# vliu15/3d-brain-tumor-segmentation

Hardware: AMD Instinct MI355X
Metric: training volumes/sec (2ch x 128^3) (higher is better)
Workload: dtype f32; 1 GPU; BASELINE configs[1]: 2ch x 128^3, batch 1 per GPU, fp32, full fwd+bwd with Dice+KL+L2 VAE loss + Dice metric + TF-form Adam; CLI-default model (base_filters=32, depth=4, groups=8, reduction=8; 42,174,773 params); parallelism=dp1, global_batch=1

## Files before the change

3d-brain-tumor-segmentation_amd/csrc/conv_igemm.hip:

```cpp
#include <stdlib.h>
#include "common.h"
#include "conv_plan.h"

#define MAXSLOT 8

int bts_prof_on();
void bts_prof_begin(int sym, double flops, hipStream_t stream);
void bts_prof_end(hipStream_t stream);

struct IgemmParams {
  const float* x;
  const float* wp;
  const float* bias;
  float* y;
  int N, Di, Hi, Wi, Cin, ldx;
  int Do, Ho, Wo;
  int Cout, ldy, Npad, KG;
  int ODa, OHa, OWa;
  int os, ooz, ooy, oox;
  int s, loz, loy, lox;
  int IZ, IY, IX;
  int lgTX, lgTY, TZ;
  int ntz, nty, ntx;
  int ntaps, flags;
// ... 1622 lines not shown
  }
  r = conv_launch(c, ch, q, stream);
  if (r == BTS_OK && ch.second) r = conv_launch(c2, ch2, q2, stream);
  if (r == BTS_OK && gn_B) *gn_B = ch.gn_B;
  return r;
}

static int conv_call_of(int dir, int kind, int N, int D, int H, int W, int Cin, int ldx, int Cout, int ldy, int flags, ConvCall& c) {
  if (N <= 0 || D <= 0 || H <= 0 || W <= 0 || Cin <= 0 || Cout <= 0 || ldx < Cin || ldy < Cout) return BTS_ERR_SHAPE;
  if (kind == BTS_CONV_K3S2 && ((D | H | W) & 1)) return BTS_ERR_SHAPE;
  const bool same = kind == BTS_CONV_K1 || kind == BTS_CONV_K3S1, half = kind == BTS_CONV_K3S2;
  const int Df = same ? D : half ? D / 2 : 2 * D, Hf = same ? H : half ? H / 2 : 2 * H, Wf = same ? W : half ? W / 2 : 2 * W;
  c = ConvCall{};
  c.geo = kind == BTS_CONV_K1 ? GEO_K1 : kind == BTS_CONV_K3S1 ? GEO_S1 : half == (dir == 0) ? GEO_DOWN : GEO_UP;
  c.N = N;
  if (dir == 0) { c.Di = D; c.Hi = H; c.Wi = W; c.Do = Df; c.Ho = Hf; c.Wo = Wf; c.Cin = Cin; c.ldx = ldx; c.Cout = Cout; c.ldy = ldy; }
  else { c.Di = Df; c.Hi = Hf; c.Wi = Wf; c.Do = D; c.Ho = H; c.Wo = W; c.Cin = Cout; c.ldx = ldy; c.Cout = Cin; c.ldy = ldx; }
  if ((flags & BTS_CONV_FLAG_SIGMOID) && dir == 0) c.flags |= IG_FLAG_SIGMOID;
  if (flags & BTS_CONV_FLAG_ACCUM) c.flags |= IG_FLAG_ACCUM;
  return BTS_OK;
}
static void conv_query_view(ConvCall& c) { c.x16 = c.y16 = c.p2_16 = c.ws16 = 1; c.ws_bytes = LONG_MAX; }
static long conv_ws_query(int dir, int kind, int N, int D, int H, int W, int Cin, int Cout) {
  ConvCall c;
  ConvChoice ch;
  if (conv_call_of(dir, kind, N, D, H, W, Cin, Cin, Cout, Cout, 0, c) != BTS_OK) return -1;
  conv_query_view(c);
  if (c.geo == GEO_UP && upm_accept(c, ch) && ch.ws > 0) return ch.ws;
  if (igemm_accept(c, ch) != BTS_OK) return -1;
  long need = ch.ws;
  if (c.geo == GEO_S1) {
    const long wn = wino_ws_need(c), w3 = w3_ws_need(c);
    need = need > wn ? need : wn;
    need = need > w3 ? need : w3;
  }
  return need;
}

extern "C" int bts_conv3d_fwd(int kind, const float* x, const float* wp_fwd, const float* bias, float* y, void* workspace,
                              long workspace_bytes, int N, int D, int H, int W, int Cin, int ldx, int Cout, int ldy,
                              int flags, hipStream_t stream) {
  ConvCall c;
  const int r = conv_call_of(0, kind, N, D, H, W, Cin, ldx, Cout, ldy, flags, c);
  if (r != BTS_OK) return r;
  if (bias) c.flags |= IG_FLAG_BIAS;
  c.ws_bytes = workspace_bytes;
  ConvPtrs q = {};
  q.x = x; q.wp = wp_fwd; q.bias = bias; q.y = y; q.ws = workspace;
  return conv_run(c, q, stream);
}
extern "C" long bts_conv3d_fwd_workspace(int kind, int N, int D, int H, int W, int Cin, int Cout) {
  return conv_ws_query(0, kind, N, D, H, W, Cin, Cout);
}

extern "C" int bts_conv3d_bwd_data(int kind, const float* dy, const float* wp_bwd, float* dx, void* workspace,
                                   long workspace_bytes, int N, int D, int H, int W, int Cin, int lddx, int Cout, int lddy,
                                   int flags, hipStream_t stream) {
  ConvCall c;
  const int r = conv_call_of(1, kind, N, D, H, W, Cin, lddx, Cout, lddy, flags, c);
  if (r != BTS_OK) return r;
  c.ws_bytes = workspace_bytes;
  ConvPtrs q = {};
  q.x = dy; q.wp = wp_bwd; q.y = dx; q.ws = workspace;
  return conv_run(c, q, stream);
}
extern "C" long bts_conv3d_bwd_data_workspace(int kind, int N, int D, int H, int W, int Cin, int Cout) {
  return conv_ws_query(1, kind, N, D, H, W, Cin, Cout);
}

extern "C" int bts_conv3d_fwd_can_fuse(int N, int D, int H, int W, int Cin, int Cout) {
  ConvCall c;
  ConvChoice ch;
  if (conv_call_of(0, BTS_CONV_K3S1, N, D, H, W, Cin, Cin, Cout, Cout, 0, c) != BTS_OK) return 0;
  conv_query_view(c);
  c.second = CONV_Y2; c.ld2 = Cout;
  return igemm_accept(c, ch) == BTS_OK;
}
extern "C" int bts_conv3d_fwd_fused2(const float* x, const float* wp_fwd, const float* bias, float* y, const float* wp2,
                                     const float* bias2, float* y2, int N, int D, int H, int W, int Cin, int ldx, int Cout,
                                     int ldy, int ldy2, hipStream_t stream) {
  ConvCall c;
  if (conv_call_of(0, BTS_CONV_K3S1, N, D, H, W, Cin, ldx, Cout, ldy, 0, c) != BTS_OK || ldy2 < Cout || !wp2 || !y2) return BTS_ERR_SHAPE;
  if (bias) c.flags |= IG_FLAG_BIAS;
  c.second = CONV_Y2; c.ld2 = ldy2;
  ConvPtrs q = {};
  q.x = x; q.wp = wp_fwd; q.bias = bias; q.y = y; q.wp2 = wp2; q.bias2 = bias2; q.y2 = y2;
  return conv_run(c, q, stream);
}

extern "C" long bts_gn_workspace(int N, long V, int C, int G, int mode);
extern "C" int bts_gn_stats(const float* x, float* mean, float* rstd, void* workspace, long workspace_bytes, int N, long V, int C,
                            int G, int mode, float eps, hipStream_t stream);
static long gnfuse_partial_bytes(int N, int Do, int Ho, int Wo, int Cout) {
  const long tiles = (long)N * ((Do + 0) ) * ((Ho + 3) / 4) * ((Wo + 7) / 8);
  return tiles * ((npad32(Cout) + 31) / 32) * 2 * (long)sizeof(double) + 64;
}
extern "C" long bts_conv3d_fwd_gn_workspace(int kind, int N, int D, int H, int W, int Cin, int Cout, int G) {
  const long cw = bts_conv3d_fwd_workspace(kind, N, D, H, W, Cin, Cout);
  if (cw < 0) return -1;
  int Do = D, Ho = H, Wo = W;
  if (kind == BTS_CONV_K3S2) { Do = D / 2; Ho = H / 2; Wo = W / 2; }
  if (kind == BTS_CONV_K3S2T) { Do = 2 * D; Ho = 2 * H; Wo = 2 * W; }
  const long gw = bts_gn_workspace(N, (long)Do * Ho * Wo, Cout, G, BTS_GN_SLAB);
  if (gw < 0) return -1;
  const long fused = ((cw + 63) & ~63L) + gnfuse_partial_bytes(N, Do, Ho, Wo, Cout);
  return fused > gw ? fused : gw;
}
static int conv_fwd_gn_impl(int kind, const float* x, const float* wp, const float* bias, float* y, const float* wp2,
                            const float* bias2, float* y2, int ldy2, void* ws, long ws_bytes, int N, int D, int H, int W, int Cin,
                            int ldx, int Cout, int G, float eps, float* mean, float* rstd, hipStream_t stream) {
  if (G <= 0 || Cout % G != 0) return BTS_ERR_SHAPE;
  if (ws == nullptr || ws_bytes < bts_conv3d_fwd_gn_workspace(kind, N, D, H, W, Cin, Cout, G)) return BTS_ERR_WORKSPACE;
  ConvCall c;
  int r = conv_call_of(0, kind, N, D, H, W, Cin, ldx, Cout, Cout, 0, c);
  if (r != BTS_OK) return r;
  if (bias) c.flags |= IG_FLAG_BIAS;
  if (wp2 != nullptr) { c.second = CONV_Y2; c.ld2 = ldy2; }
  const long cw = (bts_conv3d_fwd_workspace(kind, N, D, H, W, Cin, Cout) + 63) & ~63L;
  c.G = G; c.ws_bytes = cw;
  ConvPtrs q = {};
  q.x = x; q.wp = wp; q.bias = bias; q.y = y; q.wp2 = wp2; q.bias2 = bias2; q.y2 = y2; q.ws = ws;
  q.gnp = reinterpret_cast<double*>(reinterpret_cast<char*>(ws) + cw);
  long gnB = 0;
  r = conv_run(c, q, stream, &gnB);
  if (r != BTS_OK) return r;
  const long V = (long)c.Do * c.Ho * c.Wo;
  if (gnB > 0) return bts_gn_finalize_partials_(q.gnp, mean, rstd, N * G, gnB, (double)V * Cout / G, eps, stream);
  return bts_gn_stats(y, mean, rstd, ws, ws_bytes, N, V, Cout, G, BTS_GN_SLAB, eps, stream);
}
extern "C" int bts_conv3d_fwd_gn(int kind, const float* x, const float* wp_fwd, const float* bias, float* y, void* workspace,
                                 long workspace_bytes, int N, int D, int H, int W, int Cin, int ldx, int Cout, int G, float eps,
                                 float* mean, float* rstd, hipStream_t stream) {
  if (N <= 0 || D <= 0 || H <= 0 || W <= 0 || Cin <= 0 || Cout <= 0 || ldx < Cin) return BTS_ERR_SHAPE;
  if (((uintptr_t)workspace) & 15) return BTS_ERR_ALIGN;
  return conv_fwd_gn_impl(kind, x, wp_fwd, bias, y, nullptr, nullptr, nullptr, 0, workspace, workspace_bytes, N, D, H, W, Cin, ldx,
                          Cout, G, eps, mean, rstd, stream);
}
extern "C" int bts_conv3d_fwd_fused2_gn(const float* x, const float* wp_fwd, const float* bias, float* y, const float* wp2,
                                        const float* bias2, float* y2, void* workspace, long workspace_bytes, int N, int D, int H,
                                        int W, int Cin, int ldx, int Cout, int ldy2, int G, float eps, float* mean, float* rstd,
                                        hipStream_t stream) {
  if (N <= 0 || D <= 0 || H <= 0 || W <= 0 || Cin <= 0 || Cout <= 0 || ldx < Cin || ldy2 < Cout || !wp2 || !y2) return BTS_ERR_SHAPE;
  if (((uintptr_t)workspace) & 15) return BTS_ERR_ALIGN;
  return conv_fwd_gn_impl(BTS_CONV_K3S1, x, wp_fwd, bias, y, wp2, bias2, y2, ldy2, workspace, workspace_bytes, N, D, H, W, Cin, ldx,
                          Cout, G, eps, mean, rstd, stream);
}

extern "C" long bts_conv3d_bwd_data_pair_workspace(int N, int D, int H, int W, int Cin, int Cout) {
  const long a = bts_conv3d_bwd_data_workspace(BTS_CONV_K3S1, N, D, H, W, Cin, Cout);
  const long b = bts_conv3d_bwd_data_workspace(BTS_CONV_K1, N, D, H, W, Cin, Cout);
  if (a < 0 || b < 0) return -1;
  return a > b ? a : b;
}
extern "C" int bts_conv3d_bwd_data_pair(const float* dy, const float* wp_bwd, const float* dy2, const float* wp2_bwd, float* dx,
                                        void* workspace, long workspace_bytes, int N, int D, int H, int W, int Cin, int lddx,
                                        int Cout, int lddy, int lddy2, int flags, hipStream_t stream) {
  ConvCall c;
  if (conv_call_of(1, BTS_CONV_K3S1, N, D, H, W, Cin, lddx, Cout, lddy, flags, c) != BTS_OK || lddy2 < Cout) return BTS_ERR_SHAPE;
  const long need = conv_ws_query(1, BTS_CONV_K3S1, N, D, H, W, Cin, Cout);
  if (need < 0) return BTS_ERR_SHAPE;
  c.ws_bytes = workspace_bytes;
  ConvPtrs q = {};
  q.x = dy; q.wp = wp_bwd; q.y = dx; q.ws = workspace;
  const bool fuse = need == 0 && (Cout % 8 == 0) && (lddy2 % 4 == 0) && ((((uintptr_t)dy2) & 15) == 0) && Cin > 4 &&
                    getenv("BTS_IGEMM_NOPAIR") == nullptr;
  if (fuse) {
    c.second = CONV_X2; c.ld2 = lddy2;
    q.x2 = dy2; q.wp2 = wp2_bwd;
    return conv_run(c, q, stream);
  }
  const int r = conv_run(c, q, stream);
  if (r != BTS_OK) return r;
  return bts_conv3d_bwd_data(BTS_CONV_K1, dy2, wp2_bwd, dx, workspace, workspace_bytes, N, D, H, W, Cin, lddx, Cout, lddy2,
                             flags | BTS_CONV_FLAG_ACCUM, stream);
}

static int conv_config_query(int dir, int kind, int N, int D, int H, int W, int Cin, int Cout) {
  ConvCall c;
  ConvChoice ch;
  int r = conv_call_of(dir, kind, N, D, H, W, Cin, Cin, Cout, Cout, 0, c);
  if (r != BTS_OK) return r;
  conv_query_view(c);
  r = igemm_accept(c, ch);
  return r != BTS_OK ? r : ch.sym;
}
extern "C" int bts_conv3d_fwd_config(int kind, int N, int D, int H, int W, int Cin, int Cout) {
  return conv_config_query(0, kind, N, D, H, W, Cin, Cout);
}
extern "C" int bts_conv3d_bwd_data_config(int kind, int N, int D, int H, int W, int Cin, int Cout) {
  return conv_config_query(1, kind, N, D, H, W, Cin, Cout);
}
extern "C" int bts_conv3d_kernel(int dir, int kind, int N, int D, int H, int W, int Cin, int ldx, int Cout, int ldy, int flags, int second,
                                 int ld2, int G, int aligned, long workspace_bytes) {
  ConvCall c;
  ConvChoice ch;
  int r = conv_call_of(dir != 0, kind, N, D, H, W, Cin, ldx, Cout, ldy, flags, c);
  if (r != BTS_OK) return r;
  if (second < 0 || second > CONV_X2 || G < 0) return BTS_ERR_SHAPE;
  if (second && (c.geo != GEO_S1 || ld2 < c.Cout * (second == CONV_Y2) + c.Cin * (second == CONV_X2))) return BTS_ERR_SHAPE;
  c.second = second; c.ld2 = second ? ld2 : 0; c.G = G;
  c.x16 = aligned & 1; c.y16 = (aligned >> 1) & 1; c.p2_16 = (aligned >> 2) & 1; c.ws16 = (aligned >> 3) & 1;
  c.ws_bytes = workspace_bytes < 0 ? LONG_MAX : workspace_bytes;
  r = conv_choose(c, ch);
  return r != BTS_OK ? r : ch.sym;
}
```

3d-brain-tumor-segmentation_amd/csrc/conv_wino3.hip:

```cpp
#include <stdio.h>
#include <stdlib.h>
#include <type_traits>
#include "common.h"
#include "conv_plan.h"
#include "wino_util.h"

int bts_prof_on();
void bts_prof_begin(int sym, double flops, hipStream_t stream);
void bts_prof_end(hipStream_t stream);

struct W3Params {
  const float* x;
  const float* up;
  const float* bias;
  float* y;
  int N, D, H, W, ldx, Cout, ldy, KG;
  int ntz, nty, ntx;
  int accum;
  double* gnp;
  int gn_G, gn_zt;
  int ksplit, kg_per, Npad;
  float* part;
  int nb, ntiles, tiles_per_xcd;
  int T;
};

#define W3S 12
#define W3SX 18
#define W3LX 20
#define W3NCOL (W3SX * 6 * 2)
#define W3PL (6 * W3LX * W3S)
#define W3BUF (8 * W3PL)
#define W3NSLOT 6
#define W3EX (4 * 4 * 4 * 64 * 4)
#define W3OFF(j, k) ((((j) * W3LX) + ((k) & 1) * 10 + ((k) >> 1)) * W3S)

__global__ __launch_bounds__(256, 1) void w3_kernel(const W3Params p) {
  extern __shared__ __attribute__((aligned(16))) float lds[];
  const int tid = threadIdx.x;
  const int lane = tid & 63;
  const int wave = __builtin_amdgcn_readfirstlane(tid >> 6);
  const int h = lane >> 5, l32 = lane & 31;
  const int ptx = l32 & 7, pty = (l32 >> 3) & 1, ptz = l32 >> 4;
  const int nb_ = p.nb;
  const int xcd_ = blockIdx.x & 7;
  const int seq0 = (blockIdx.x >> 3) * p.T;
  int tiles_left = p.ntiles - xcd_ * p.tiles_per_xcd;
  if (tiles_left > p.tiles_per_xcd) tiles_left = p.tiles_per_xcd;
  const int items_here = tiles_left * nb_;
  if (seq0 >= items_here) return;

  struct Item { int n, tz, ty, tx, cb; };
  auto decode = [&](int seq) {
    Item it;
    it.cb = seq % nb_;
    int b = xcd_ * p.tiles_per_xcd + seq / nb_;
    it.tx = b % p.ntx; b /= p.ntx;
    it.ty = b % p.nty; b /= p.nty;
    it.tz = b % p.ntz;
    it.n = b / p.ntz;
    return it;
  };
  auto advance = [&](Item& it) {
    if (++it.cb < nb_) return;
    it.cb = 0;
    if (++it.tx < p.ntx) return;
    it.tx = 0;
    if (++it.ty < p.nty) return;
    it.ty = 0;
    if (++it.tz < p.ntz) return;
    it.tz = 0;
    ++it.n;
  };

  const int s_q = tid & 1, s_vy = (tid >> 1) / W3SX, s_vx = (tid >> 1) - s_vy * W3SX;
  const bool s_on = tid < W3NCOL;
  const unsigned gcol = (unsigned)((s_vy * p.W + s_vx) * p.ldx + s_q * 4) * 4u;
  const unsigned gplane = (unsigned)(p.H * p.W * p.ldx) * 4u;
  const int lcol = (s_vy * W3LX + (s_vx & 1) * 10 + (s_vx >> 1)) * W3S + s_q * 4;
  __amdgpu_buffer_rsrc_t xr, wr, wr_n;
  unsigned goff[W3NSLOT];
  auto setup_x = [&](const Item& it) {
    const int iz0 = it.tz * 4 - 1, iy0 = it.ty * 4 - 1, ix0 = it.tx * 16 - 1;
    const float* xorg = p.x + ((((long)it.n * p.D + iz0) * p.H + iy0) * p.W + ix0) * (long)p.ldx;
    xr = __builtin_amdgcn_make_buffer_rsrc((void*)xorg, 0, 0x7fffffff, 0x00020000);
    const bool col_in = s_on && (unsigned)(iy0 + s_vy) < (unsigned)p.H && (unsigned)(ix0 + s_vx) < (unsigned)p.W;
#pragma unroll
    for (int i = 0; i < W3NSLOT; ++i) goff[i] = (col_in && (unsigned)(iz0 + i) < (unsigned)p.D) ? gcol + (unsigned)i * gplane : 0x80000000u;
  };
  auto wdesc = [&](const Item& it) {
    return __builtin_amdgcn_make_buffer_rsrc((void*)(p.up + (long)it.cb * p.KG * (64 * 256)), 0, 0x7fffffff, 0x00020000);
  };
  const __amdgpu_buffer_rsrc_t br =
      __builtin_amdgcn_make_buffer_rsrc((void*)p.bias, 0, (p.bias && p.ksplit <= 1) ? (unsigned)p.Cout * 4u : 0u, 0x00020000);
  auto bias_of = [&](const Item& it) {
    return __builtin_bit_cast(float, __builtin_amdgcn_raw_buffer_load_b32(br, tid < 32 ? (unsigned)(it.cb * 32 + tid) * 4u : 0x80000000u, 0, 0));
  };

  int st0 = 0, st1 = p.KG;
  if (p.ksplit > 1) {
    st0 = blockIdx.z * p.kg_per;
    st1 = st0 + p.kg_per;
    if (st1 > p.KG) st1 = p.KG;
  }

  const int offP = (ptz * 4 + wave) * W3PL + (2 * pty * W3LX + ptx) * W3S + h * 4;
  const unsigned wlane = (unsigned)((h * 32 + l32) * 16);
  const unsigned wwave = (unsigned)(wave * 16 * 1024);

  f32x16 acc[4][4];
  f32x4 pre[W3NSLOT];
  auto fetch = [&](unsigned soff) {
#pragma unroll
    for (int i = 0; i < W3NSLOT; ++i) pre[i] = bufload(xr, goff[i], soff);
  };
  auto commit = [&](float* buf) {
    if (s_on) {
      float* o = buf + lcol;
#pragma unroll
      for (int zp = 0; zp < 2; ++zp) {
        const f32x4 d0 = pre[2 * zp], d1 = pre[2 * zp + 1], d2 = pre[2 * zp + 2], d3 = pre[2 * zp + 3];
        *reinterpret_cast<f32x4*>(o + (zp * 4 + 0) * W3PL) = sub4(d0, d2);
        *reinterpret_cast<f32x4*>(o + (zp * 4 + 1) * W3PL) = add4(d1, d2);
        *reinterpret_cast<f32x4*>(o + (zp * 4 + 2) * W3PL) = sub4(d2, d1);
        *reinterpret_cast<f32x4*>(o + (zp * 4 + 3) * W3PL) = sub4(d1, d3);
      }
    }
  };
  f32x4 aw[4][4];
  auto wload = [&](f32x4 (&dst)[4], const __amdgpu_buffer_rsrc_t d, int st, int b) {
    const unsigned so = (unsigned)(st * (64 * 1024) + b * 4096) + wwave;
#pragma unroll
    for (int e = 0; e < 4; ++e) dst[e] = bufload(d, wlane + e * 1024, so);
  };
  f32x4 c[4][4], v[2][4], t[4];
  auto rd_row = [&](const float* lb, int j) {
#pragma unroll
    for (int k = 0; k < 4; ++k) c[j][k] = *reinterpret_cast<const f32x4*>(lb + offP + W3OFF(j, k));
  };
  float* const ex = lds + 2 * W3BUF;
  float* const bsh = ex + W3EX;
  double* const gsh = reinterpret_cast<double*>(bsh + 64);
  float bias_v = 0.f;

  auto stage = [&](auto first_tag, int st, int par, unsigned f_soff, const __amdgpu_buffer_rsrc_t wt, int stn, int bslot) {
    constexpr bool FIRST = decltype(first_tag)::value;
    const float* lb = lds + par * W3BUF;
    const float* ln = lds + (par ^ 1) * W3BUF;
    {
      wload(aw[2], wr, st, 0);
      rd_row(lb, 0);
#pragma unroll
      for (int k = 0; k < 4; ++k) t[k] = sub4(c[2][k], c[1][k]);
      wino_yt(t, v[1]);
      wino_mfma16<FIRST>(v[0], aw[0], acc[1]);
      WINO_SCHED_GROUP();
      __builtin_amdgcn_sched_barrier(0);
      asm volatile("s_nop 1" ::: "memory");
    }
    {
      wload(aw[3], wr, st, 3);
      rd_row(lb, 3);
#pragma unroll
      for (int k = 0; k < 4; ++k) t[k] = sub4(c[0][k], c[2][k]);
      wino_yt(t, v[0]);
      wino_mfma16<FIRST>(v[1], aw[1], acc[2]);
      WINO_SCHED_GROUP();
      __builtin_amdgcn_sched_barrier(0);
      asm volatile("s_nop 1" ::: "memory");
    }
    {
      wload(aw[0], wt, stn, 1);
#pragma unroll
      for (int k = 0; k < 4; ++k) t[k] = sub4(c[1][k], c[3][k]);
      wino_yt(t, v[1]);
      wino_mfma16<FIRST>(v[0], aw[2], acc[0]);
      WINO_SCHED_GROUP();
      __builtin_amdgcn_sched_barrier(0);
      commit(lds + (par ^ 1) * W3BUF);
      if (FIRST && tid < 32) bsh[bslot * 32 + tid] = bias_v;
      __syncthreads();
      fetch(f_soff);
    }
    {
      wload(aw[1], wt, stn, 2);
      rd_row(ln, 1);
      rd_row(ln, 2);
#pragma unroll
      for (int k = 0; k < 4; ++k) t[k] = add4(c[1][k], c[2][k]);
      wino_yt(t, v[0]);
      wino_mfma16<FIRST>(v[1], aw[3], acc[3]);
      WINO_SCHED_GROUP();
      __builtin_amdgcn_sched_barrier(0);
      asm volatile("s_nop 1" ::: "memory");
    }
  };

  const bool raw = p.ksplit > 1;
  const int ld = raw ? p.Npad : p.ldy;
  const int clim = raw ? p.Npad : p.Cout;
  const bool acc_in = p.accum && !raw;
  auto finish = [&](const Item& o, int bslot) {
    const float* obase = raw ? p.part + ((long)blockIdx.z * p.N + o.n) * p.D * p.H * p.W * (long)p.Npad
                             : p.y + (long)o.n * p.D * p.H * p.W * (long)p.ldy;
    const __amdgpu_buffer_rsrc_t yr = __builtin_amdgcn_make_buffer_rsrc((void*)obase, 0, 0x7fffffff, 0x00020000);
    asm volatile("s_nop 15\n\ts_nop 15\n\ts_nop 15\n\ts_nop 15\n\ts_nop 15" ::: "memory");
#pragma unroll
    for (int g = 0; g < 4; ++g) {
      f32x4 tq[4][2];
#pragma unroll
      for (int b = 0; b < 4; ++b) {
        f32x4 q[4];
#pragma unroll
        for (int k = 0; k < 4; ++k)
          q[k] = f32x4{acc_rd(acc[b][k][4 * g]), acc_rd(acc[b][k][4 * g + 1]), acc_rd(acc[b][k][4 * g + 2]), acc_rd(acc[b][k][4 * g + 3])};
        tq[b][0] = add4(add4(q[0], q[1]), q[2]);
        tq[b][1] = sub4(sub4(q[1], q[2]), q[3]);
      }
#pragma unroll
      for (int ox = 0; ox < 2; ++ox) {
        const f32x4 m0 = add4(add4(tq[0][ox], tq[1][ox]), tq[2][ox]);
        const f32x4 m1 = sub4(sub4(tq[1][ox], tq[2][ox]), tq[3][ox]);
        *reinterpret_cast<f32x4*>(ex + (((wave * 4 + g) * 4 + 0 + ox) * 64 + lane) * 4) = m0;
        *reinterpret_cast<f32x4*>(ex + (((wave * 4 + g) * 4 + 2 + ox) * 64 + lane) * 4) = m1;
      }
      __builtin_amdgcn_sched_barrier(0);
    }
    __syncthreads();
    f32x2 gn_s2 = {0.f, 0.f}, gn_q2 = {0.f, 0.f};
    const bool gn_on = p.gnp != nullptr;
    {
      const int oy = wave >> 1, ox = wave & 1;
      const int zb = o.tz * 4 + 2 * ptz, yy = o.ty * 4 + 2 * pty + oy, xx = o.tx * 16 + 2 * ptx + ox;
      unsigned yo[2];
#pragma unroll
      for (int oz = 0; oz < 2; ++oz) {
        const bool ok = xx < p.W && yy < p.H && (zb + oz) < p.D;
        yo[oz] = ok ? (unsigned)(((((zb + oz) * p.H + yy) * p.W + xx) * ld + o.cb * 32 + 4 * h) * 4) : 0x80000000u;
      }
      f32x4 old[4][2];
#pragma unroll
      for (int g = 0; g < 4; ++g)
#pragma unroll
        for (int oz = 0; oz < 2; ++oz) {
          const bool cok = o.cb * 32 + 8 * g + 4 * h < clim;
          old[g][oz] = bufload(yr, (acc_in && cok) ? yo[oz] + 32u * g : 0x80000000u, 0);
        }
#pragma unroll
      for (int g = 0; g < 4; ++g) {
        f32x4 m[4];
#pragma unroll
        for (int a = 0; a < 4; ++a) m[a] = *reinterpret_cast<const f32x4*>(ex + (((a * 4 + g) * 4 + wave) * 64 + lane) * 4);
        const f32x4 bq = *reinterpret_cast<const f32x4*>(bsh + bslot * 32 + 8 * g + 4 * h);
        f32x4 ov[2];
        ov[0] = add4(add4(add4(m[0], m[1]), m[2]), bq);
        ov[1] = add4(sub4(sub4(m[1], m[2]), m[3]), bq);
        const bool cok = o.cb * 32 + 8 * g + 4 * h < clim;
#pragma unroll
        for (int oz = 0; oz < 2; ++oz) {
          const unsigned off = cok ? yo[oz] : 0x80000000u;
          const bool live = off != 0x80000000u;
          f32x4 w = ov[oz];
          if (gn_on) {
            const f32x4 tt = live ? w : f32x4{0.f, 0.f, 0.f, 0.f};
            gn_s2 = pk_add(pk_add(gn_s2, tt.xy), tt.zw);
            gn_q2 = pk_fma(tt.zw, tt.zw, pk_fma(tt.xy, tt.xy, gn_q2));
          }
          w = add4(w, old[g][oz]);
          __builtin_amdgcn_raw_buffer_store_b128(__builtin_bit_cast(u32x4, w), yr, off + 32u * g, 0, 0);
        }
      }
    }
    {
      double s0 = 0.0, s1 = 0.0;
      const double* dst = nullptr;
      if (gn_on) {
        const double ds = wave_sum_f64((double)gn_s2.x + (double)gn_s2.y), dq = wave_sum_f64((double)gn_q2.x + (double)gn_q2.y);
        if (lane == 0) { gsh[wave * 2] = ds; gsh[wave * 2 + 1] = dq; }
        __syncthreads();
        const int gn_g = o.tz / p.gn_zt;
        const long B = (long)p.gn_zt * p.nty * p.ntx * nb_;
        const long gn_slot = (((long)(o.tz - gn_g * p.gn_zt) * p.nty + o.ty) * p.ntx + o.tx) * nb_ + o.cb;
        dst = p.gnp + (((long)o.n * p.gn_G + gn_g) * B + gn_slot) * 2;
        s0 = gsh[0] + gsh[2] + gsh[4] + gsh[6];
        s1 = gsh[1] + gsh[3] + gsh[5] + gsh[7];
      }
      const __amdgpu_buffer_rsrc_t gr = __builtin_amdgcn_make_buffer_rsrc((void*)dst, 0, gn_on ? 16 : 0, 0x00020000);
      struct D2 { double a, b; } d2{s0, s1};
      __builtin_amdgcn_raw_buffer_store_b128(__builtin_bit_cast(u32x4, d2), gr, (gn_on && tid == 0) ? 0u : 0x80000000u, 0, 0);
    }
  };

  Item cur = decode(seq0), nxt = cur;
  setup_x(cur);
  wr = wdesc(cur);
  wr_n = wr;
  fetch((unsigned)st0 * 32u);
  wload(aw[0], wr, st0, 1);
  wload(aw[1], wr, st0, 2);
  bias_v = bias_of(cur);
  {
    const __amdgpu_buffer_rsrc_t none = __builtin_amdgcn_make_buffer_rsrc((void*)p.y, 0, 0, 0x00020000);
    f32x4 z = {0.f, 0.f, 0.f, 0.f};
#pragma unroll
    for (int i = 0; i < 8; ++i) z += bufload(none, 0x80000000u + 16u * i, 0);
#pragma unroll
    for (int i = 0; i < 9; ++i) __builtin_amdgcn_raw_buffer_store_b128(__builtin_bit_cast(u32x4, z), none, 0x80000000u + 16u * i, 0, 0);
    const float dummy = bias_of(cur);
    asm volatile("" ::"v"(dummy));
  }
  commit(lds);
  __syncthreads();
  fetch(st0 + 1 < st1 ? (unsigned)(st0 + 1) * 32u : 0x80000000u);
  rd_row(lds, 1);
  rd_row(lds, 2);
#pragma unroll
  for (int k = 0; k < 4; ++k) t[k] = add4(c[1][k], c[2][k]);
  wino_yt(t, v[0]);
  __builtin_amdgcn_sched_barrier(0);
  asm volatile("s_nop 3" ::: "memory");

  int par = 0;
  for (int it = 0; it < p.T; ++it) {
    const bool have_next = (it + 1 < p.T) && (seq0 + it + 1 < items_here);
    const Item out = cur;
    float bias_n = 0.f;
    if (have_next) {
      advance(nxt);
      wr_n = wdesc(nxt);
    }
    bias_n = bias_of(nxt);
    auto run = [&](auto first_tag, int st) {
      if (st + 2 == st1 && have_next) setup_x(nxt);
      const int f = st + 2;
      const unsigned f_soff = f < st1 ? (unsigned)f * 32u : (have_next ? (unsigned)(st0 + f - st1) * 32u : 0x80000000u);
      const bool last = st + 1 == st1;
      stage(first_tag, st, par, f_soff, last ? wr_n : wr, last ? st0 : st + 1, it & 1);
      par ^= 1;
    };
    run(std::true_type{}, st0);
    for (int st = st0 + 1; st < st1; ++st) run(std::false_type{}, st);
    finish(out, it & 1);
    if (!have_next) break;
    cur = nxt;
    wr = wr_n;
    bias_v = bias_n;
  }
}

static int w3_enabled() {
  const char* e = getenv("BTS_WINO");
  if (e && atoi(e) == 0) return 0;
  e = getenv("BTS_W3");
  return e ? atoi(e) : 1;
}

static bool w3_plan(W3Plan& q, int N, int D, int H, int W, int Cin, int Cout) {
  if (Cin % 8 != 0 || Cout % 4 != 0 || Cout < 16) return false;
  if (W < 12 || H < 4 || D < 4) return false;
  q.ntz = (D + 3) / 4;
  q.nty = (H + 3) / 4;
  q.ntx = (W + 15) / 16;
  q.nb = (Cout + 31) / 32;
  q.wgs = (long)N * q.ntz * q.nty * q.ntx * q.nb;
  if (q.wgs > 0x7fffffffL / 16) return false;
  wino_split(q, N, D, H, W, Cin, 384, 512);
  return true;
}
long w3_ws_need(const ConvCall& c) {
  W3Plan q;
  return w3_enabled() && w3_plan(q, c.N, c.Di, c.Hi, c.Wi, c.Cin, c.Cout) ? q.need : 0;
}
bool w3_accept(const ConvCall& c, ConvChoice& ch) {
  if (!w3_enabled() || !wino_call_ok(c) || !w3_plan(ch.w, c.N, c.Di, c.Hi, c.Wi, c.Cin, c.Cout)) return false;
  ch.sym = 27;
  return wino_plan_ok(c, ch);
}

int bts_w3_launch_(const ConvCall& c, const ConvChoice& ch, const ConvPtrs& q, hipStream_t stream) {
  const W3Plan& pl = ch.w;
  const int N = c.N, D = c.Di, H = c.Hi, W = c.Wi, Cin = c.Cin, Cout = c.Cout;
  const float* bias = (c.flags & IG_FLAG_BIAS) ? q.bias : nullptr;
  const int accum = (c.flags & IG_FLAG_ACCUM) ? 1 : 0;
  W3Params p;
  p.x = q.x; p.up = q.wp + 75L * ((long)(Cin / 8) * 2 * (pl.nb * 32) * 4); p.bias = bias; p.y = q.y;
  p.N = N; p.D = D; p.H = H; p.W = W; p.ldx = c.ldx; p.Cout = Cout; p.ldy = c.ldy; p.KG = Cin / 8;
  p.ntz = pl.ntz; p.nty = pl.nty; p.ntx = pl.ntx;
  p.accum = accum;
  p.ksplit = pl.ksplit; p.kg_per = pl.kg_per; p.Npad = pl.nb * 32; p.part = reinterpret_cast<float*>(q.ws);
  p.nb = pl.nb; p.ntiles = N * pl.ntz * pl.nty * pl.ntx; p.tiles_per_xcd = (p.ntiles + 7) / 8;
  p.gnp = pl.gn_zt ? q.gnp : nullptr; p.gn_G = pl.gn_zt ? c.G : 0; p.gn_zt = pl.gn_zt ? pl.gn_zt : 1;
  static bool attr_done = false;
  const size_t shmem = (2 * W3BUF + W3EX + 64 + 16) * sizeof(float);
  {
    const long items = (long)p.tiles_per_xcd * pl.nb;
    p.T = 1;
    if (pl.ksplit == 1 && p.KG >= 2) {
      long best = -1;
      for (int t = 1; t <= 8; ++t) {
        const long rounds = ((items + t - 1) / t + 31) / 32;
        const long cost = rounds * (8L * t + 1);
        if (best < 0 || cost <= best) { best = cost; p.T = t; }
      }
      const char* e = getenv("BTS_W3_T");
      if (e && atoi(e) > 0) p.T = atoi(e);
    }
  }
  const long wgs_per_xcd = ((long)p.tiles_per_xcd * pl.nb + p.T - 1) / p.T;
  if (!attr_done) {
    hipError_t e = hipFuncSetAttribute(reinterpret_cast<const void*>(w3_kernel), hipFuncAttributeMaxDynamicSharedMemorySize, 160 * 1024);
    if (e != hipSuccess) return (int)e;
    attr_done = true;
  }
  const double flops = 2.0 * 27 * Cin * Cout * (double)N * D * H * W;
  const bool prof = bts_prof_on();
  if (prof) bts_prof_begin(27, flops, stream);
  (void)hipGetLastError();
  hipLaunchKernelGGL(w3_kernel, dim3((unsigned)(8L * wgs_per_xcd), 1, pl.ksplit), dim3(256), shmem, stream, p);
  if (prof) bts_prof_end(stream);
  BTS_LAUNCH_CHECK();
  if (pl.ksplit == 1) return BTS_OK;
  return bts_igemm_reduce_(p.part, bias, q.y, (long)N * D * H * W, Cout, p.Npad, c.ldy, pl.ksplit, bias != nullptr, accum, stream);
}
```

include/bts_hip.h:

```cpp
#ifndef BTS_HIP_H
#define BTS_HIP_H
#include <stdint.h>
#ifdef __cplusplus
extern "C" {
#endif

typedef struct ihipStream_t* bts_stream_t;

#define BTS_OK 0
#define BTS_ERR_SHAPE (-1)
#define BTS_ERR_ALIGN (-2)
#define BTS_ERR_UNSUPPORTED (-3)
#define BTS_ERR_WORKSPACE (-4)
#define BTS_ERR_RCCL_BASE (-100)

#define BTS_CONV_K1 0
#define BTS_CONV_K3S1 1
#define BTS_CONV_K3S2 2
#define BTS_CONV_K3S2T 3
#define BTS_ROLE_FWD 0
#define BTS_ROLE_BWD_DATA 1
#define BTS_CONV_FLAG_SIGMOID 1
#define BTS_CONV_FLAG_ACCUM 2

#define BTS_GN_SLAB 0
#define BTS_GN_CHANNEL 1


long bts_conv_packed_floats(int kind, int role, int Cin, int Cout);
int bts_conv_pack(int kind, int role, const float* w, float* wp, int Cin_ref, int Cout, int Cin_slab, int dup_start,
                  int dup_shift, bts_stream_t stream);
long bts_conv_pack_desc_bytes(void);
long bts_conv_pack_desc(void* host_table, int index, long first_block, int kind, int role, const float* w, float* wp,
                        int Cin_ref, int Cout, int Cin_slab, int dup_start, int dup_shift);
int bts_conv_pack_batch(const void* table_dev, const void* table_host, int n, long total_blocks, bts_stream_t stream);
long bts_conv_pack_generation(void);
int bts_conv_pack_forget(const float* wp);
long bts_conv3d_fwd_workspace(int kind, int N, int D, int H, int W, int Cin, int Cout);
int bts_conv3d_fwd(int kind, const float* x, const float* wp_fwd, const float* bias, float* y, void* workspace,
                   long workspace_bytes, int N, int D, int H, int W, int Cin, int ldx, int Cout, int ldy, int flags,
                   bts_stream_t stream);
int bts_conv3d_fwd_can_fuse(int N, int D, int H, int W, int Cin, int Cout);
int bts_conv3d_fwd_fused2(const float* x, const float* wp_fwd, const float* bias, float* y, const float* wp2,
                          const float* bias2, float* y2, int N, int D, int H, int W, int Cin, int ldx, int Cout, int ldy,
                          int ldy2, bts_stream_t stream);
long bts_conv3d_bwd_data_workspace(int kind, int N, int D, int H, int W, int Cin, int Cout);
int bts_conv3d_bwd_data(int kind, const float* dy, const float* wp_bwd, float* dx, void* workspace, long workspace_bytes,
                        int N, int D, int H, int W, int Cin, int lddx, int Cout, int lddy, int flags, bts_stream_t stream);
int bts_conv3d_fwd_config(int kind, int N, int D, int H, int W, int Cin, int Cout);
int bts_conv3d_bwd_data_config(int kind, int N, int D, int H, int W, int Cin, int Cout);
int bts_conv3d_kernel(int dir, int kind, int N, int D, int H, int W, int Cin, int ldx, int Cout, int ldy, int flags, int second,
                      int ld2, int G, int aligned, long workspace_bytes);
long bts_conv3d_bwd_weight_workspace(int kind, int N, int D, int H, int W, int Cin, int Cout);
int bts_conv3d_bwd_weight(int kind, const float* x, const float* dy, float* dw, float* db, void* workspace,
                          long workspace_bytes, int N, int D, int H, int W, int Cin, int ldx, int Cout, int lddy,
                          int dup_start, int dup_shift, int accumulate, bts_stream_t stream);
int bts_conv3d_bwd_weight_form(int kind, int N, int D, int H, int W, int Cin, int ldx, int Cout, int lddy, int aligned);

long bts_gn_workspace(int N, long V, int C, int G, int mode);
long bts_gn_bwd_workspace(int N, long V, int C, int G, int mode);
int bts_gn_stats(const float* x, float* mean, float* rstd, void* workspace, long workspace_bytes, int N, long V, int C,
                 int G, int mode, float eps, bts_stream_t stream);
int bts_gn_apply(const float* x, float* y, const float* gamma, const float* beta, const float* mean, const float* rstd,
                 int N, long V, int C, int ldy, int G, int mode, int relu, bts_stream_t stream);
int bts_gn_bwd(const float* x, const float* dy, float* dx, const float* gamma, const float* beta, const float* mean,
               const float* rstd, float* dgamma, float* dbeta, void* workspace, long workspace_bytes, int N, long V, int C,
               int lddy, int G, int mode, int relu, int accumulate_params, bts_stream_t stream);

long bts_colsum_workspace(int N, long rows, int C);
int bts_colsum(const float* x, float* out, void* workspace, long workspace_bytes, int N, long rows, int C, int ld,
               float scale, int sum_over_n, int accumulate, bts_stream_t stream);
int bts_se_mlp_fwd(const float* gap, const float* w1, const float* w2, float* h, float* ch, int N, int F, int R,
                   bts_stream_t stream);
int bts_block_epilogue_fwd(const float* res, const float* c2, float* out, float* sp, const float* wsp, const float* ch,
                           const float* gamma, const float* beta, const float* mean, const float* rstd, int N, long V,
                           int F, int ldo, int G, int mode, bts_stream_t stream);
long bts_se_bwd_workspace(int N, long V, int F, int R);
int bts_se_bwd(const float* dout, const float* res, const float* sp, const float* gap, const float* h, const float* ch,
               const float* w1, const float* w2, const float* wsp, float* dres, float* ds, float* dgap, float* dw1,
               float* dw2, float* dwsp, void* workspace, long workspace_bytes, int N, long V, int F, int R, int lddo,
               int accumulate_params, bts_stream_t stream);

long bts_block_bwd_workspace(int N, long V, int F, int R, int G);
int bts_block_bwd(const float* dout, int lddo, const float* res, const float* c2, const float* sp, const float* gap, const float* h,
                  const float* ch, const float* w1, const float* w2, const float* wsp, const float* gamma, const float* beta,
                  const float* mean, const float* rstd, float* dres, float* dc2, float* ds, float* dgap, float* dw1, float* dw2,
                  float* dwsp, float* dgamma, float* dbeta, void* workspace, long workspace_bytes, int N, long V, int F, int R, int G,
                  int accumulate_gate_params, int accumulate_norm_params, bts_stream_t stream);

int bts_dropout_mask(uint8_t* mask, long n, float rate, uint64_t seed, bts_stream_t stream);
int bts_dropout_apply(const float* x, const uint8_t* mask, float* y, long n, float rate, bts_stream_t stream);
int bts_normal(float* out, long n, uint64_t seed, bts_stream_t stream);
int bts_vae_sample_fwd(const float* proj, const float* eps, float* z, int N, int L, bts_stream_t stream);
int bts_vae_sample_bwd(const float* proj, const float* eps, const float* dz, float* dproj, int N, int L, bts_stream_t stream);
int bts_fill(float* p, long n, float v, bts_stream_t stream);
int bts_axpy(float* y, const float* x, long n, float a, bts_stream_t stream);
int bts_add_strided(float* dst, const float* src, long rows, int C, int ldd, int lds_, int accumulate, bts_stream_t stream);
int bts_scalar_lincomb(float* out, const float* a, const float* b, float ca, float cb, bts_stream_t stream);
int bts_relu_bwd(const float* y, const float* dy, float* dx, long n, bts_stream_t stream);
int bts_sigmoid_bwd(const float* y, const float* dy, float* dx, long rows, int C, int ldy, int lddy, bts_stream_t stream);

long bts_dense_workspace(int N, int in, int out);
int bts_dense_fwd(const float* x, const float* w, const float* bias, float* y, void* workspace, long workspace_bytes, int N,
                  int in, int out, int relu, bts_stream_t stream);
int bts_dense_bwd(const float* x, const float* w, const float* g, float* dx, float* dw, float* db, int N, int in, int out,
                  int accumulate_dx, int accumulate_params, bts_stream_t stream);

long bts_loss_workspace(void);
int bts_loss_sums(const float* y_pred, const float* y, const float* x, const float* y_vae, const float* proj, double* sums,
                  void* workspace, long workspace_bytes, int N, long V, int C, int ldp, int ldy, int Cx, int ldx, int ldv,
                  int Lz, bts_stream_t stream);
int bts_loss_value(const double* sums, float* loss, float* parts, int C, int has_vae, bts_stream_t stream);
int bts_loss_bwd(const float* y_pred, const float* y, const float* x, const float* y_vae, const float* proj,
                 const double* sums, const float* gscale, float* dlogit, float* dyvae, float* dproj, int N, long V, int C,
                 int ldp, int ldy, int Cx, int ldx, int ldv, int Lz, int through_sigmoid, bts_stream_t stream);
int bts_dice_metric_sums(const float* y_true, const float* y_pred, uint8_t* labels, double* table, int N, long V, int W,
                         int C, int ldt, int ldp, int channels_last_axes, bts_stream_t stream);
int bts_dice_metric_value(const double* table, float* out, int W, int C, int channels_last_axes, bts_stream_t stream);
long bts_l2_workspace(void);
int bts_l2_reg_fwd(const float* params, const long* off, const long* len, const float* coef, int nranges, float* out,
                   void* workspace, long workspace_bytes, bts_stream_t stream);
int bts_l2_reg_bwd(const float* params, float* grads, const long* off, const long* len, const float* coef, int nranges,
                   const float* gscale, bts_stream_t stream);

int bts_adam_tf_step(float* p, const float* g, float* m, float* v, long n, float lr_t, float beta1, float beta2, float eps,
                     float gmul, bts_stream_t stream);
int bts_grad_nonfinite(const float* g, long n, int* flag, bts_stream_t stream);
int bts_adam_tf_step_guarded(float* p, const float* g, float* m, float* v, long n, float lr_t, float beta1, float beta2, float eps,
                             float gmul, const int* skip, bts_stream_t stream);

long bts_conv3d_bwd_data_pair_workspace(int N, int D, int H, int W, int Cin, int Cout);
int bts_conv3d_bwd_data_pair(const float* dy, const float* wp_bwd, const float* dy2, const float* wp2_bwd, float* dx,
                             void* workspace, long workspace_bytes, int N, int D, int H, int W, int Cin, int lddx, int Cout,
                             int lddy, int lddy2, int flags, bts_stream_t stream);

long bts_conv3d_fwd_gn_workspace(int kind, int N, int D, int H, int W, int Cin, int Cout, int G);
int bts_conv3d_fwd_gn(int kind, const float* x, const float* wp_fwd, const float* bias, float* y, void* workspace,
                      long workspace_bytes, int N, int D, int H, int W, int Cin, int ldx, int Cout, int G, float eps, float* mean,
                      float* rstd, bts_stream_t stream);
int bts_conv3d_fwd_fused2_gn(const float* x, const float* wp_fwd, const float* bias, float* y, const float* wp2,
                             const float* bias2, float* y2, void* workspace, long workspace_bytes, int N, int D, int H, int W,
                             int Cin, int ldx, int Cout, int ldy2, int G, float eps, float* mean, float* rstd,
                             bts_stream_t stream);

int bts_maxpool2_fwd(const float* x, float* y, uint8_t* idx, int N, int D, int H, int W, int C, int ldx, int ldy,
                     bts_stream_t stream);
int bts_maxpool2_bwd(const float* dy, const uint8_t* idx, float* dx, int N, int D, int H, int W, int C, int lddy, int lddx,
                     int accumulate, bts_stream_t stream);
int bts_upsample2_fwd(const float* x, float* y, int N, int D, int H, int W, int C, int ldx, int ldy, bts_stream_t stream);
int bts_upsample2_bwd(const float* dy, float* dx, int N, int D, int H, int W, int C, int lddy, int lddx, int accumulate,
                      bts_stream_t stream);

int bts_flip_affine(const float* src, float* dst, const float* mean, const float* stdv, int N, int D, int H, int W, int C,
                    int flip_mask, float scale, int accumulate, bts_stream_t stream);
int bts_tta_finish(const float* prob, const float* bmask, float* y, uint8_t* labels, long nvox, int C, float threshold,
                   bts_stream_t stream);

int bts_spline_prefilter3d(const float* src, float* dst, int D, int H, int W, int C, bts_stream_t stream);
int bts_zoom3d(const float* coef, float* dst, float* bmask, const float* mean, const float* stdv, int Din, int Hin, int Win,
               int Dout, int Hout, int Wout, int C, int Dpad, int Hpad, int Wpad, int order, bts_stream_t stream);

int bts_skull_strip(const float* x, const float* p, const float* m, float* xo, float* mo, int Da, int Ha, int Wa, int D, int H, int W,
                    int Db, int Hb, int Wb, int C, bts_stream_t stream);
int bts_label_confusion(const uint8_t* truth, const uint8_t* pred, long nvox, int K, long* counts, bts_stream_t stream);
int bts_region_surface(const uint8_t* lab, uint8_t* surf, long* count, int D, int H, int W, int K, int class_mask, bts_stream_t stream);
int bts_edt3d_sq(const uint8_t* feat, double* dist2, int D, int H, int W, double sd, double sh, double sw, bts_stream_t stream);
long bts_masked_select_workspace(int nranks);
int bts_masked_select(const double* v, const uint8_t* mask, long n, const long* ranks, int nranks, double* out, void* work,
                      bts_stream_t stream);
int bts_components3d(const uint8_t* lab, int* comp, int D, int H, int W, int K, int class_mask, int connectivity, bts_stream_t stream);
int bts_component_sizes(const int* comp, long n, int* size, long* ncomp, bts_stream_t stream);
int bts_component_largest(const int* size, long n, uint64_t* key, bts_stream_t stream);
int bts_components_apply(uint8_t* lab, const int* comp, const int* size, const uint64_t* key, long n, int min_voxels, int largest_only,
                         int fill, long* removed_voxels, long* removed_components, bts_stream_t stream);
int bts_region_relabel(uint8_t* lab, long n, int K, int class_mask, int fill, const long* confusion, long limit, long* changed,
                       bts_stream_t stream);
long bts_dilate3d_workspace(int D, int H, int W, int iterations, int fuse);
int bts_dilate3d(const uint8_t* lab, uint8_t* out, int D, int H, int W, int K, int class_mask, int connectivity, int iterations, int fuse,
                 void* work, bts_stream_t stream);
long bts_lesion_pairs_table_bytes(long capacity);
int bts_lesion_pairs(const int* td_comp, const uint8_t* truth, const int* pred_comp, long n, int K, int class_mask, int* lesion_vox,
                     void* table, long capacity, long* status, bts_stream_t stream);
int bts_component_boxes(const int* comp, int D, int H, int W, const int* roots, int nroots, int* boxes, bts_stream_t stream);
int bts_lesion_crop(const int* td_comp, const uint8_t* truth, const int* pred_comp, int D, int H, int W, int K, int class_mask, int d0,
                    int h0, int w0, int d1, int h1, int w1, int td_root, const int* roots, int nroots, uint8_t* g, uint8_t* m,
                    bts_stream_t stream);

long bts_window_batch_max(void);
int bts_window_gather(const float* x, float* out, int D, int H, int W, int C, int R0, int R1, int R2, int B, const int* starts,
                      const int* flips, const float* mean, const float* stdv, bts_stream_t stream);
int bts_window_accumulate(const float* pred, float* acc, const float* nz, const float* ny, const float* nx, int n0, int n1, int n2, int D,
                          int H, int W, int K, int R0, int R1, int R2, int B, const int* starts, const int* flips, const int* rows,
                          float scale, bts_stream_t stream);
int bts_window_occupancy(const float* mask, const int* starts, int* counts, int n0, int n1, int n2, int D, int H, int W, int R0, int R1,
                         int R2, bts_stream_t stream);

long bts_channel_moments_workspace(int C);
int bts_channel_moments(const float* x, float* mean, float* var, void* workspace, long workspace_bytes, long nvox, int C,
                        int ld, bts_stream_t stream);
int bts_augment_crop(const float* x, const float* y, const float* var, float* xo, float* yo, int S0, int S1, int S2, int C,
                     int T0, int T1, int T2, int o0, int o1, int o2, int flip_mask, const float* shift, const float* scale,
                     int out_ch, bts_stream_t stream);
long bts_augment_batch_max(void);
int bts_augment_batch(const float* const* x, const float* const* y, const float* const* var, float* xo, float* yo, int N, int S0,
                      int S1, int S2, int C, int T0, int T1, int T2, const int* offsets, const int* flips, const float* shift,
// ... 159 lines not shown
```

Baseline: 28.29 volumes/s.

## Fuse the 1x1 second conv into the Winograd 3x3 backward-data epilogue

After: 28.89 volumes/s, median of 6. 1.02x the previous value.

```diff
diff --git a/3d-brain-tumor-segmentation_amd/csrc/conv_igemm.hip b/3d-brain-tumor-segmentation_amd/csrc/conv_igemm.hip
--- a/3d-brain-tumor-segmentation_amd/csrc/conv_igemm.hip
+++ b/3d-brain-tumor-segmentation_amd/csrc/conv_igemm.hip
@@ -1798,20 +1798,36 @@
   if (a < 0 || b < 0) return -1;
   return a > b ? a : b;
 }
+static int pair_call_of(int N, int D, int H, int W, int Cin, int lddx, int Cout, int lddy, int lddy2, int flags, bool dy2_16, ConvCall& c) {
+  if (conv_call_of(1, BTS_CONV_K3S1, N, D, H, W, Cin, lddx, Cout, lddy, flags, c) != BTS_OK || lddy2 < Cout) return BTS_ERR_SHAPE;
+  const long need = conv_ws_query(1, BTS_CONV_K3S1, N, D, H, W, Cin, Cout);
+  if (need < 0) return BTS_ERR_SHAPE;
+  const bool fuse = need == 0 && (Cout % 8 == 0) && (lddy2 % 4 == 0) && dy2_16 && Cin > 4 && getenv("BTS_IGEMM_NOPAIR") == nullptr;
+  if (fuse) { c.second = CONV_X2; c.ld2 = lddy2; }
+  return fuse;
+}
+extern "C" int bts_conv3d_bwd_data_pair_launches(int N, int D, int H, int W, int Cin, int lddx, int Cout, int lddy, int lddy2, int flags,
+                                                 int aligned, long workspace_bytes) {
+  ConvCall c;
+  ConvChoice ch;
+  const int fuse = pair_call_of(N, D, H, W, Cin, lddx, Cout, lddy, lddy2, flags, (aligned >> 2) & 1, c);
+  if (fuse < 0) return fuse;
+  if (!fuse) return 2;
+  c.x16 = aligned & 1; c.y16 = (aligned >> 1) & 1; c.p2_16 = 1; c.ws16 = (aligned >> 3) & 1;
+  c.ws_bytes = workspace_bytes < 0 ? LONG_MAX : workspace_bytes;
+  const int r = conv_choose(c, ch);
+  return r != BTS_OK ? r : ch.second ? 2 : 1;
+}
 extern "C" int bts_conv3d_bwd_data_pair(const float* dy, const float* wp_bwd, const float* dy2, const float* wp2_bwd, float* dx,
                                         void* workspace, long workspace_bytes, int N, int D, int H, int W, int Cin, int lddx,
                                         int Cout, int lddy, int lddy2, int flags, hipStream_t stream) {
   ConvCall c;
-  if (conv_call_of(1, BTS_CONV_K3S1, N, D, H, W, Cin, lddx, Cout, lddy, flags, c) != BTS_OK || lddy2 < Cout) return BTS_ERR_SHAPE;
-  const long need = conv_ws_query(1, BTS_CONV_K3S1, N, D, H, W, Cin, Cout);
-  if (need < 0) return BTS_ERR_SHAPE;
+  const int fuse = pair_call_of(N, D, H, W, Cin, lddx, Cout, lddy, lddy2, flags, (((uintptr_t)dy2) & 15) == 0, c);
+  if (fuse < 0) return fuse;
   c.ws_bytes = workspace_bytes;
   ConvPtrs q = {};
   q.x = dy; q.wp = wp_bwd; q.y = dx; q.ws = workspace;
-  const bool fuse = need == 0 && (Cout % 8 == 0) && (lddy2 % 4 == 0) && ((((uintptr_t)dy2) & 15) == 0) && Cin > 4 &&
-                    getenv("BTS_IGEMM_NOPAIR") == nullptr;
   if (fuse) {
-    c.second = CONV_X2; c.ld2 = lddy2;
     q.x2 = dy2; q.wp2 = wp2_bwd;
     return conv_run(c, q, stream);
   }
diff --git a/3d-brain-tumor-segmentation_amd/csrc/conv_wino3.hip b/3d-brain-tumor-segmentation_amd/csrc/conv_wino3.hip
--- a/3d-brain-tumor-segmentation_amd/csrc/conv_wino3.hip
+++ b/3d-brain-tumor-segmentation_amd/csrc/conv_wino3.hip
@@ -23,6 +23,9 @@
   float* part;
   int nb, ntiles, tiles_per_xcd;
   int T;
+  const float* x2;
+  const float* wp2;
+  int ld2, KG2;
 };
 
 #define W3S 12
@@ -35,6 +38,7 @@
 #define W3EX (4 * 4 * 4 * 64 * 4)
 #define W3OFF(j, k) ((((j) * W3LX) + ((k) & 1) * 10 + ((k) >> 1)) * W3S)
 
+template <bool X2>
 __global__ __launch_bounds__(256, 1) void w3_kernel(const W3Params p) {
   extern __shared__ __attribute__((aligned(16))) float lds[];
   const int tid = threadIdx.x;
@@ -200,10 +204,34 @@
   const int ld = raw ? p.Npad : p.ldy;
   const int clim = raw ? p.Npad : p.Cout;
   const bool acc_in = p.accum && !raw;
+  f32x4 wf[2][2], xf[2][2][2];
+  __amdgpu_buffer_rsrc_t x2r, w2r;
+  unsigned x2o[2], w2o = 0x80000000u;
+  auto x2_req = [&](int b, int kg0) {
+#pragma unroll
+    for (int k = 0; k < 2; ++k)
+#pragma unroll
+      for (int oz = 0; oz < 2; ++oz) xf[b][k][oz] = bufload(x2r, kg0 + k < p.KG2 ? x2o[oz] : 0x80000000u, (unsigned)(kg0 + k) * 32u);
+  };
+  auto w2_req = [&](int b, int kg0) {
+#pragma unroll
+    for (int k = 0; k < 2; ++k) wf[b][k] = bufload(w2r, kg0 + k < p.KG2 ? w2o : 0x80000000u, (unsigned)(kg0 + k) * (unsigned)(p.Npad * 32));
+  };
   auto finish = [&](const Item& o, int bslot) {
     const float* obase = raw ? p.part + ((long)blockIdx.z * p.N + o.n) * p.D * p.H * p.W * (long)p.Npad
                              : p.y + (long)o.n * p.D * p.H * p.W * (long)p.ldy;
     const __amdgpu_buffer_rsrc_t yr = __builtin_amdgcn_make_buffer_rsrc((void*)obase, 0, 0x7fffffff, 0x00020000);
+    if (X2) {
+      const int yy = o.ty * 4 + 2 * pty + (wave >> 1), xx = o.tx * 16 + 2 * ptx + (wave & 1), zb = o.tz * 4 + 2 * ptz;
+      x2r = __builtin_amdgcn_make_buffer_rsrc((void*)(p.x2 + (long)o.n * p.D * p.H * p.W * (long)p.ld2), 0, 0x7fffffff, 0x00020000);
+      w2r = __builtin_amdgcn_make_buffer_rsrc((void*)p.wp2, 0, (unsigned)p.KG2 * (unsigned)(p.Npad * 32), 0x00020000);
+#pragma unroll
+      for (int oz = 0; oz < 2; ++oz)
+        x2o[oz] = (xx < p.W && yy < p.H && (zb + oz) < p.D) ? (unsigned)(((((zb + oz) * p.H + yy) * p.W + xx) * p.ld2 + 4 * h) * 4) : 0x80000000u;
+      w2o = (o.cb * 32 + l32 < p.Cout) ? (unsigned)((h * p.Npad + o.cb * 32 + l32) * 16) : 0x80000000u;
+      x2_req(0, 0);
+      x2_req(1, 2);
+    }
     asm volatile("s_nop 15\n\ts_nop 15\n\ts_nop 15\n\ts_nop 15\n\ts_nop 15" ::: "memory");
 #pragma unroll
     for (int g = 0; g < 4; ++g) {
@@ -226,6 +254,11 @@
       }
       __builtin_amdgcn_sched_barrier(0);
     }
+    if (X2) {
+      w2_req(0, 0);
+      w2_req(1, 2);
+      __builtin_amdgcn_sched_barrier(0);
+    }
     __syncthreads();
     f32x2 gn_s2 = {0.f, 0.f}, gn_q2 = {0.f, 0.f};
     const bool gn_on = p.gnp != nullptr;
@@ -246,6 +279,28 @@
           const bool cok = o.cb * 32 + 8 * g + 4 * h < clim;
           old[g][oz] = bufload(yr, (acc_in && cok) ? yo[oz] + 32u * g : 0x80000000u, 0);
         }
+      f32x16 a2[2];
+      if (X2) {
+        const f32x16 zero16 = {0.f, 0.f, 0.f, 0.f, 0.f, 0.f, 0.f, 0.f, 0.f, 0.f, 0.f, 0.f, 0.f, 0.f, 0.f, 0.f};
+        for (int kg0 = 0; kg0 < p.KG2; kg0 += 4) {
+#pragma unroll
+          for (int b = 0; b < 2; ++b) {
+            if (b == 0 || kg0 + 2 < p.KG2) {
+#pragma unroll
+              for (int k = 0; k < 2; ++k)
+#pragma unroll
+                for (int j = 0; j < 4; ++j)
+#pragma unroll
+                  for (int oz = 0; oz < 2; ++oz)
+                    a2[oz] = __builtin_amdgcn_mfma_f32_32x32x2f32(wf[b][k][j], xf[b][k][oz][j], (kg0 | b | k | j) ? a2[oz] : zero16, 0, 0, 0);
+            }
+            if (kg0 + 4 < p.KG2) {
+              w2_req(b, kg0 + 4 + 2 * b);
+              x2_req(b, kg0 + 4 + 2 * b);
+            }
+          }
+        }
+      }
 #pragma unroll
       for (int g = 0; g < 4; ++g) {
         f32x4 m[4];
@@ -261,6 +316,7 @@
           const unsigned off = cok ? yo[oz] : 0x80000000u;
           const bool live = off != 0x80000000u;
           f32x4 w = ov[oz];
+          if (X2) w = add4(w, f32x4{a2[oz][4 * g], a2[oz][4 * g + 1], a2[oz][4 * g + 2], a2[oz][4 * g + 3]});
           if (gn_on) {
             const f32x4 tt = live ? w : f32x4{0.f, 0.f, 0.f, 0.f};
             gn_s2 = pk_add(pk_add(gn_s2, tt.xy), tt.zw);
@@ -303,7 +359,7 @@
     const __amdgpu_buffer_rsrc_t none = __builtin_amdgcn_make_buffer_rsrc((void*)p.y, 0, 0, 0x00020000);
     f32x4 z = {0.f, 0.f, 0.f, 0.f};
 #pragma unroll
-    for (int i = 0; i < 8; ++i) z += bufload(none, 0x80000000u + 16u * i, 0);
+    for (int i = 0; i < (X2 ? 20 : 8); ++i) z += bufload(none, 0x80000000u + 16u * i, 0);
 #pragma unroll
     for (int i = 0; i < 9; ++i) __builtin_amdgcn_raw_buffer_store_b128(__builtin_bit_cast(u32x4, z), none, 0x80000000u + 16u * i, 0, 0);
     const float dummy = bias_of(cur);
@@ -374,7 +430,12 @@
 bool w3_accept(const ConvCall& c, ConvChoice& ch) {
   if (!w3_enabled() || !wino_call_ok(c) || !w3_plan(ch.w, c.N, c.Di, c.Hi, c.Wi, c.Cin, c.Cout)) return false;
   ch.sym = 27;
-  return wino_plan_ok(c, ch);
+  if (!wino_plan_ok(c, ch)) return false;
+  const long nvox = (long)c.N * c.Di * c.Hi * c.Wi;
+  if (c.second == CONV_X2 && ch.w.ksplit == 1 && c.ld2 % 4 == 0 && c.p2_16 &&
+      nvox >= conv_env_long("BTS_IGEMM_K1S_MIN", 256 * 256) && ((long)c.Di * c.Hi * c.Wi + 64) * (long)c.ld2 * 4 < 0x7fffffffL)
+    ch.second = 0;
+  return true;
 }
 
 int bts_w3_launch_(const ConvCall& c, const ConvChoice& ch, const ConvPtrs& q, hipStream_t stream) {
@@ -390,6 +451,8 @@
   p.ksplit = pl.ksplit; p.kg_per = pl.kg_per; p.Npad = pl.nb * 32; p.part = reinterpret_cast<float*>(q.ws);
   p.nb = pl.nb; p.ntiles = N * pl.ntz * pl.nty * pl.ntx; p.tiles_per_xcd = (p.ntiles + 7) / 8;
   p.gnp = pl.gn_zt ? q.gnp : nullptr; p.gn_G = pl.gn_zt ? c.G : 0; p.gn_zt = pl.gn_zt ? pl.gn_zt : 1;
+  const bool x2 = c.second == CONV_X2 && ch.second == 0;
+  p.x2 = x2 ? q.x2 : nullptr; p.wp2 = x2 ? q.wp2 : nullptr; p.ld2 = x2 ? c.ld2 : 0; p.KG2 = x2 ? Cin / 8 : 0;
   static bool attr_done = false;
   const size_t shmem = (2 * W3BUF + W3EX + 64 + 16) * sizeof(float);
   {
@@ -408,7 +471,9 @@
   }
   const long wgs_per_xcd = ((long)p.tiles_per_xcd * pl.nb + p.T - 1) / p.T;
   if (!attr_done) {
-    hipError_t e = hipFuncSetAttribute(reinterpret_cast<const void*>(w3_kernel), hipFuncAttributeMaxDynamicSharedMemorySize, 160 * 1024);
+    hipError_t e = hipFuncSetAttribute(reinterpret_cast<const void*>(w3_kernel<false>), hipFuncAttributeMaxDynamicSharedMemorySize, 160 * 1024);
+    if (e != hipSuccess) return (int)e;
+    e = hipFuncSetAttribute(reinterpret_cast<const void*>(w3_kernel<true>), hipFuncAttributeMaxDynamicSharedMemorySize, 160 * 1024);
     if (e != hipSuccess) return (int)e;
     attr_done = true;
   }
@@ -416,7 +481,8 @@
   const bool prof = bts_prof_on();
   if (prof) bts_prof_begin(27, flops, stream);
   (void)hipGetLastError();
-  hipLaunchKernelGGL(w3_kernel, dim3((unsigned)(8L * wgs_per_xcd), 1, pl.ksplit), dim3(256), shmem, stream, p);
+  if (x2) hipLaunchKernelGGL(w3_kernel<true>, dim3((unsigned)(8L * wgs_per_xcd), 1, 1), dim3(256), shmem, stream, p);
+  else hipLaunchKernelGGL(w3_kernel<false>, dim3((unsigned)(8L * wgs_per_xcd), 1, pl.ksplit), dim3(256), shmem, stream, p);
   if (prof) bts_prof_end(stream);
   BTS_LAUNCH_CHECK();
   if (pl.ksplit == 1) return BTS_OK;
diff --git a/include/bts_hip.h b/include/bts_hip.h
--- a/include/bts_hip.h
+++ b/include/bts_hip.h
@@ -51,6 +51,8 @@
 int bts_conv3d_bwd_data_config(int kind, int N, int D, int H, int W, int Cin, int Cout);
 int bts_conv3d_kernel(int dir, int kind, int N, int D, int H, int W, int Cin, int ldx, int Cout, int ldy, int flags, int second,
                       int ld2, int G, int aligned, long workspace_bytes);
+int bts_conv3d_bwd_data_pair_launches(int N, int D, int H, int W, int Cin, int lddx, int Cout, int lddy, int lddy2, int flags,
+                                      int aligned, long workspace_bytes);
 long bts_conv3d_bwd_weight_workspace(int kind, int N, int D, int H, int W, int Cin, int Cout);
 int bts_conv3d_bwd_weight(int kind, const float* x, const float* dy, float* dw, float* db, void* workspace,
                           long workspace_bytes, int N, int D, int H, int W, int Cin, int ldx, int Cout, int lddy,
```
